# unilight/seq2seq-vc

Measured on AMD Instinct MI355X. Metric: mel-frames/sec (train), higher is better.
Workload: dtype bf16; 1 GPU; VTN egs/arctic/vc1 (vtn.v1.yaml) training step: fwd+Seq2SeqLoss+bwd+clip+Adam+WarmupLR; batch_per_gpu=32, global_batch=32, T_src=256, T_tgt=256, mel_dim=80, parallelism=dp1, split_backward=False, hip_graph=True, backward_stages=1

## Files before the change

### include/s2svc_hip.h

```cpp
#ifndef S2SVC_HIP_H
#define S2SVC_HIP_H
#include <stdint.h>
#ifdef __cplusplus
extern "C" {
#endif

const char* s2svc_last_error(void);
int s2svc_abi_version(void);
int s2svc_launch_floor(int workgroups, int threads, void* sink_1024_words, void* stream);

int s2svc_event_create(void** out );
int s2svc_event_destroy(void* ev);
int s2svc_event_record(void* ev, void* stream);
int s2svc_stream_wait_event(void* stream, void* ev);

enum { S2SVC_LAYOUT_KC = 0,
       S2SVC_LAYOUT_RC = 1 };
enum { S2SVC_OP_DENSE = 0,
       S2SVC_OP_CONV1D = 1,
       S2SVC_OP_CONV2D_S2 = 2,
       S2SVC_OP_TCONV2D_S2 = 3 };

typedef struct {
  const void* ptr;
// ... 121 lines not shown
  int32_t k;
  int32_t reserved_;
} s2svc_scalar_terms;
int s2svc_weighted_sum(const s2svc_scalar_terms* terms , float* out, void* stream);
int s2svc_weighted_sum_bwd(const s2svc_scalar_terms* grads , const float* g, void* stream);
int s2svc_scalars_axpy(const s2svc_scalar_terms* terms , float beta, float* acc, void* stream);
int s2svc_fill_zero(void* p, int64_t nbytes, void* stream);
int s2svc_seed_advance(uint64_t* seed, uint64_t inc, void* stream);
int s2svc_pad_cols(int dtype, int64_t rows, int N, int ldo, const void* in, void* out, void* stream);
int s2svc_decoder_input(int out_dtype, int B, int Tin, int r, int D, int64_t ys_batch_stride, const float* ys, void* out, void* stream);
int s2svc_append_eos(int B, int T, int64_t ldx, const int64_t* xs, const int32_t* lens, int64_t eos, int64_t pad, int64_t* out, void* stream);
int s2svc_copy_rows(int dtype, int64_t rows, int D, int64_t lds, const void* src, void* out, void* stream);
int s2svc_stop_labels(int B, int T, int64_t ld_labels, const float* labels, const int32_t* lens, float* out, void* stream);
int s2svc_add_n(int dtype, int64_t n, int k, const void* x0, const void* x1, const void* x2, const void* x3, void* out, void* stream);
int s2svc_add_head_bias(int dtype, int64_t rows, int D, const void* q, const float* u, const float* v, void* qu, void* qv,
                        void* stream);
int s2svc_add_head_bias_ld(int dtype, int64_t rows, int D, const void* q, int64_t ldq, const float* u, const float* v, void* qu,
                           void* qv, void* stream);
int s2svc_add_rows(int dtype, int64_t rows, int D, const void* a, int64_t lda, const void* b, int64_t ldb, void* out, int64_t ldo,
                   void* stream);
int s2svc_glu_fwd(int dtype, int64_t rows, int C, const void* x, void* y, void* stream);
int s2svc_glu_bwd(int dtype, int64_t rows, int C, const void* x, const void* dy, void* dx, void* stream);
int s2svc_cast(int in_dtype, int out_dtype, int64_t n, const void* x, void* y, void* stream);
int s2svc_gather3(int in_dtype, int out_dtype, int n0, int n1, int n2, int64_t s0, int64_t s1, int64_t s2, int64_t off,
                  const void* in, void* out, void* stream);
typedef struct s2svc_gather3_job {
  const void* in;
  void* out;
  int64_t s0, s1, s2, off;
  int32_t n0, n1, n2;
  int32_t out_dtype;
} s2svc_gather3_job;
int s2svc_gather3_grouped(const s2svc_gather3_job* jobs , int n, void* stream);
int s2svc_permute_inner(int n, int A, int B, const float* src, float* dst, int accumulate, void* stream);
int s2svc_rowscale(int dtype, int64_t rows, int D, const void* x, const float* s, void* out, void* stream);

int s2svc_conv_in1_fwd(int dtype, int B, int Tn, int Fn, int O, const void* x, const float* w, const float* bias, void* y,
                       void* stream);
int s2svc_conv_in1_wgrad(int dtype, int B, int Tn, int Fn, int O, const void* x, const void* dy, const void* y, float* dw,
                         float* db, int accumulate, float* partial, int max_chunks, void* stream);
int s2svc_col2im_s2(int dtype, int B, int T1, int F1, int C, int T2, int F2, const void* dcols, void* dx, void* stream);
int s2svc_interp_nearest(int dtype, int B, int Tin, int Tout, int C, const void* x, void* y, const int32_t* ext_in,
                         const int32_t* ext_out, void* stream);
int s2svc_interp_nearest_bwd(int dtype, int B, int Tin, int Tout, int C, const void* dy, void* dx, const int32_t* ext_in,
                             const int32_t* ext_out, void* stream);
int s2svc_dwconv(int dtype, int B, int Tn, int C, int ks, int dil, const void* x, const float* w, const float* bias,
                 void* y, int flip, void* stream);
int s2svc_dwconv_add(int dtype, int B, int Tn, int C, int ks, int dil, const void* x, const float* w, const float* bias,
                     const void* add, void* y, int flip, void* stream);
int s2svc_dwconv_wgrad(int dtype, int B, int Tn, int C, int ks, int dil, const void* x, const void* dy, float* dw,
                       int accumulate, float* ws, int ws_chunks, void* stream);

int s2svc_convmod_supported(int C, int ks);
int s2svc_convmod_fwd(int B, int Tn, int C, int ks, const void* y2, const float* w, const float* bias, void* z, float eps,
                      float momentum, float* mean, float* rstd, float* run_mean, float* run_var, int64_t* num_batches, float* ws,
                      const int32_t* vlens, void* stream);
int s2svc_bn_swish_apply(int64_t rows, int C, const void* z, const float* mean, const float* rstd, const float* gamma,
                         const float* beta, void* out, int Tn, const int32_t* vlens, void* stream);
int s2svc_convmod_bwd(int B, int Tn, int C, int ks, const void* da, const void* z, const void* y2, const float* w, const float* mean,
                      const float* rstd, const float* gamma, const float* beta, void* dy2, float* sdy, float* sdyx,
                      float* dgamma_acc, float* dbeta_acc, float* ws_stats, float* ws_w, const int32_t* vlens, void* stream);
int s2svc_convmod_wgrad_final(int C, int ks, int chunks, const float* ws_w, float* dw, float* db, int accumulate, void* stream);

int s2svc_bn_stats_vec(int rows, int C, const void* x, float eps, float momentum, float* mean, float* rstd, float* run_mean,
                       float* run_var, int64_t* num_batches, float* ws, int Tn, const int32_t* vlens, void* stream);
int s2svc_bn_act_apply_vec(int rows, int C, const void* x, const float* mean, const float* rstd, const float* gamma, const float* beta,
// ... 195 lines not shown
```

### seq2seq_vc_amd/_lib.py

```python
import ctypes
import os
import subprocess
import sys
from concurrent.futures import ThreadPoolExecutor

_HERE = os.path.dirname(os.path.abspath(__file__))
CSRC = os.path.join(_HERE, "csrc")
LIB_PATH = os.environ.get("S2SVC_LIB") or os.path.join(CSRC, "libs2svc_hip.so")
HIPCC = os.environ.get("HIPCC", "/opt/rocm/bin/hipcc")
ARCH = "gfx950"


def sources():
    return sorted(f for f in os.listdir(CSRC) if f.endswith(".hip"))


DEBUG_EXEC_LIB_PATH = os.path.join(CSRC, "libs2svc_hip_dbgexec.so")


def build_library(force=False, verbose=True, debug_exec=False):
    lib_path = DEBUG_EXEC_LIB_PATH if debug_exec else LIB_PATH
    if not debug_exec and os.environ.get("S2SVC_LIB"):
        lib_path = os.path.join(CSRC, "libs2svc_hip.so")
    srcs = [os.path.join(CSRC, f) for f in sources()]
# ... 49 lines not shown
    if verbose:
        print("[s2svc build]", " ".join(cmd), file=sys.stderr)
    subprocess.run(cmd, check=True)
    return TORCH_OPS_LIB_PATH


c_i32, c_i64, c_f32, c_u64, c_vp = ctypes.c_int32, ctypes.c_int64, ctypes.c_float, ctypes.c_uint64, ctypes.c_void_p


class Operand(ctypes.Structure):
    _fields_ = [("ptr", c_vp), ("ld", c_i64), ("layout", c_i32), ("mode", c_i32), ("C", c_i32), ("T", c_i32),
                ("pad", c_i32), ("T1", c_i32), ("F1", c_i32), ("T2", c_i32), ("F2", c_i32), ("bs0", c_i64),
                ("bs1", c_i64), ("zero_padded", c_i32), ("reserved_", c_i32)]


class GemmDesc(ctypes.Structure):
    _fields_ = [("A", Operand), ("B", Operand), ("C", c_vp), ("ldc", c_i64), ("cbs0", c_i64), ("cbs1", c_i64),
                ("c_dtype", c_i32), ("bias", c_vp), ("res", c_vp), ("ldr", c_i64), ("rbs0", c_i64), ("rbs1", c_i64),
                ("M", c_i32), ("N", c_i32), ("K", c_i32), ("nb0", c_i32), ("nb1", c_i32), ("act", c_i32),
                ("alpha", c_f32), ("dtype", c_i32), ("accumulate", c_i32), ("splitk", c_i32), ("ws", c_vp),
                ("a_rowsum", c_vp), ("a_rowsum_ws", c_vp), ("a_rowsum_accumulate", c_i32), ("tile_hint", c_i32),
                ("emask", c_vp), ("ldm", c_i64), ("drop_p", c_f32), ("emask_mode", c_i32), ("seed_base", c_vp),
                ("seed_off", c_u64), ("c_map", c_i32), ("cm_T1", c_i32), ("cm_F1", c_i32), ("cm_Tc", c_i32), ("cm_Fc", c_i32),
                ("cm_pt", c_i32), ("cm_pf", c_i32), ("reserved3_", c_i32), ("c_pre", c_vp)]


class ScalarTerms(ctypes.Structure):
    _fields_ = [("x", c_vp * 8), ("n", c_i32 * 8), ("w", c_f32 * 8), ("k", c_i32), ("reserved_", c_i32)]


class Gather3Job(ctypes.Structure):
    _fields_ = [("in_", c_vp), ("out", c_vp), ("s0", c_i64), ("s1", c_i64), ("s2", c_i64), ("off", c_i64), ("n0", c_i32),
                ("n1", c_i32), ("n2", c_i32), ("out_dtype", c_i32)]


class ColreduceItem(ctypes.Structure):
    _fields_ = [("dy", c_vp), ("x", c_vp), ("mean", c_vp), ("rstd", c_vp), ("out_sum", c_vp), ("out_dot", c_vp), ("ws", c_vp),
                ("dtype", c_i32), ("rows", c_i32), ("D", c_i32), ("mode", c_i32), ("accumulate", c_i32), ("ws_chunks", c_i32),
                ("scale", c_f32), ("reserved_", c_i32)]


_SIGS = {
    "s2svc_gemm": [ctypes.POINTER(GemmDesc), c_vp],
    "s2svc_gemm_grouped_ok": [c_vp],
    "s2svc_tconv2d_weights": [c_i32, c_i32, c_vp, c_vp, c_vp],
    "s2svc_gemm_grouped": [c_vp, c_i32, c_i32, c_vp],
    "s2svc_gemm_grouped_batched": [c_vp, c_i32, c_vp],
    "s2svc_gemm_wgrad_ok": [c_vp],
    "s2svc_gemm_wgrad_grouped": [c_vp, c_i32, c_vp, c_vp],
    "s2svc_gemm_wgrad_grouped_bg": [c_vp, c_i32, c_vp, c_vp, c_i32],
    "s2svc_gemm_set_w8": [c_i32, c_i32],
    "s2svc_gemm_set_8ph": [c_i32],
    "s2svc_launch_floor": [c_i32, c_i32, c_vp, c_vp],
    "s2svc_event_create": [c_vp],
    "s2svc_event_destroy": [c_vp],
    "s2svc_event_record": [c_vp, c_vp],
    "s2svc_stream_wait_event": [c_vp, c_vp],
    "s2svc_decode_ln_linear_supported": [c_i32, c_i32, c_i32],
    "s2svc_decode_ln_linear": [ctypes.POINTER(GemmDesc), c_vp, c_vp, c_f32, c_vp, c_i64, c_vp],
    "s2svc_length_regulate_index": [c_i32, c_i32, c_i32, c_vp, c_vp, c_vp, c_vp, c_vp],
    "s2svc_length_regulate_fwd": [c_i32, c_i32, c_i32, c_i32, c_i32, c_vp, c_vp, c_f32, c_vp, c_vp],
    "s2svc_length_regulate_bwd": [c_i32, c_i32, c_i32, c_i32, c_i32, c_vp, c_vp, c_vp, c_vp, c_vp],
    "s2svc_attn_durations": [c_i32, c_i32, c_i32, c_vp, c_vp, c_vp, c_vp, c_vp],
    "s2svc_layernorm_fwd": [c_i32, c_i32, c_i32, c_vp, c_vp, c_f32, c_f32, c_vp, c_u64, c_vp, c_vp, c_f32, c_vp, c_vp, c_vp, c_vp, c_vp],
    "s2svc_layernorm_bwd": [c_i32, c_i32, c_i32, c_vp, c_vp, c_vp, c_vp, c_vp, c_vp, c_f32, c_f32, c_vp, c_u64, c_vp, c_vp, c_vp],
    "s2svc_layernorm_bwd_pg_chunks": [c_i32, c_i32, c_i32, c_vp, c_vp, c_vp, c_vp, c_vp, c_vp],
# ... 2 lines not shown
    "s2svc_colreduce": [c_i32, c_i32, c_i32, c_i32, c_vp, c_vp, c_vp, c_vp, c_f32, c_vp, c_vp, c_i32, c_vp, c_i32, c_i32, c_vp, c_vp],
    "s2svc_bn_finalize": [c_i32, c_i32, c_f32, c_f32, c_vp, c_vp, c_vp, c_vp, c_vp, c_vp, c_i32, c_i32, c_vp, c_vp],
    "s2svc_rstd_from_var": [c_i32, c_f32, c_vp, c_vp, c_vp],
    "s2svc_bn_apply": [c_i32, c_i64, c_i32, c_vp, c_vp, c_vp, c_vp, c_vp, c_i32, c_f32, c_vp, c_u64, c_vp, c_vp, c_i32, c_vp, c_vp],
    "s2svc_bn_bwd": [c_i32, c_i64, c_i32, c_vp, c_vp, c_vp, c_vp, c_vp, c_vp, c_vp, c_i32, c_vp, c_i32, c_vp, c_vp],
    "s2svc_bn_stats": [c_i32, c_i32, c_i32, c_vp, c_f32, c_f32, c_vp, c_vp, c_vp, c_vp, c_vp, c_vp, c_i32, c_i32, c_vp, c_vp],
    "s2svc_attn_softmax_fwd": [c_i32, c_i32, c_i32, c_i32, c_i32, c_i32, c_vp, c_vp, c_i32, c_i32, c_i32, c_f32, c_vp, c_i32, c_f32,
                               c_vp, c_u64, c_vp, c_vp, c_vp],
    "s2svc_attn_softmax_bwd": [c_i32, c_i32, c_i32, c_i32, c_i32, c_i32, c_vp, c_vp, c_vp, c_f32, c_f32, c_vp, c_u64, c_vp, c_vp, c_i32,
                               c_i32, c_i32, c_vp],
    "s2svc_act_dropout_fwd": [c_i32, c_i64, c_vp, c_i32, c_f32, c_vp, c_u64, c_vp, c_vp],
    "s2svc_act_dropout_bwd": [c_i32, c_i64, c_vp, c_vp, c_i32, c_f32, c_vp, c_u64, c_vp, c_vp],
    "s2svc_posenc_fwd": [c_i32, c_i64, c_i32, c_i32, c_vp, c_f32, c_vp, c_vp, c_f32, c_vp, c_u64, c_vp, c_vp],
    "s2svc_posenc_bwd": [c_i32, c_i64, c_i32, c_i32, c_vp, c_f32, c_vp, c_f32, c_vp, c_u64, c_vp, c_vp, c_vp, c_vp],
    "s2svc_axpby": [c_i32, c_i64, c_f32, c_vp, c_f32, c_vp, c_vp, c_vp],
    "s2svc_add_n": [c_i32, c_i64, c_i32, c_vp, c_vp, c_vp, c_vp, c_vp, c_vp],
    "s2svc_weighted_sum": [ctypes.POINTER(ScalarTerms), c_vp, c_vp],
    "s2svc_weighted_sum_bwd": [ctypes.POINTER(ScalarTerms), c_vp, c_vp],
    "s2svc_scalars_axpy": [ctypes.POINTER(ScalarTerms), c_f32, c_vp, c_vp],
    "s2svc_fill_zero": [c_vp, c_i64, c_vp],
    "s2svc_seed_advance": [c_vp, c_u64, c_vp],
    "s2svc_pad_cols": [c_i32, c_i64, c_i32, c_i32, c_vp, c_vp, c_vp],
    "s2svc_decoder_input": [c_i32, c_i32, c_i32, c_i32, c_i32, c_i64, c_vp, c_vp, c_vp],
    "s2svc_stop_labels": [c_i32, c_i32, c_i64, c_vp, c_vp, c_vp, c_vp],
    "s2svc_append_eos": [c_i32, c_i32, c_i64, c_vp, c_vp, c_i64, c_i64, c_vp, c_vp],
    "s2svc_copy_rows": [c_i32, c_i64, c_i32, c_i64, c_vp, c_vp, c_vp],
    "s2svc_add_head_bias": [c_i32, c_i64, c_i32, c_vp, c_vp, c_vp, c_vp, c_vp, c_vp],
    "s2svc_add_head_bias_ld": [c_i32, c_i64, c_i32, c_vp, c_i64, c_vp, c_vp, c_vp, c_vp, c_vp],
    "s2svc_add_rows": [c_i32, c_i64, c_i32, c_vp, c_i64, c_vp, c_i64, c_vp, c_i64, c_vp],
    "s2svc_glu_fwd": [c_i32, c_i64, c_i32, c_vp, c_vp, c_vp],
    "s2svc_glu_bwd": [c_i32, c_i64, c_i32, c_vp, c_vp, c_vp, c_vp],
    "s2svc_cast": [c_i32, c_i32, c_i64, c_vp, c_vp, c_vp],
    "s2svc_gather3_grouped": [c_vp, c_i32, c_vp],
    "s2svc_permute_inner": [c_i32, c_i32, c_i32, c_vp, c_vp, c_i32, c_vp],
    "s2svc_gather3": [c_i32, c_i32, c_i32, c_i32, c_i32, c_i64, c_i64, c_i64, c_i64, c_vp, c_vp, c_vp],
    "s2svc_mas": [c_i32, c_i32, c_i32, c_vp, c_vp, c_vp, c_vp, c_vp, c_vp, c_vp, c_vp],
    "s2svc_mas_binloss_bwd": [c_i32, c_i32, c_i32, c_vp, c_vp, c_vp, c_vp, c_vp],
    "s2svc_seq_loss_fwd": [c_i32, c_i32, c_i32, c_i32, c_vp, c_vp, c_vp, c_vp, c_vp, c_vp, c_f32, c_vp, c_vp, c_vp],
    "s2svc_seq_loss_bwd": [c_i32, c_i32, c_i32, c_i32, c_vp, c_vp, c_vp, c_vp, c_vp, c_vp, c_f32, c_vp, c_vp, c_vp, c_vp,
                           c_vp, c_vp, c_vp],
    "s2svc_guided_attn_loss_fwd": [c_i32, c_i32, c_i32, c_i32, c_i32, c_vp, c_vp, c_vp, c_f32, c_f32, c_vp, c_vp, c_vp],
    "s2svc_guided_attn_loss_bwd": [c_i32, c_i32, c_i32, c_i32, c_i32, c_vp, c_vp, c_f32, c_f32, c_vp, c_vp, c_vp, c_vp],
    "s2svc_adam_step": [c_i64, c_vp, c_vp, c_vp, c_vp, c_vp, c_f32, c_f32, c_f32, c_f32, c_f32, c_f32, c_vp, c_vp, c_vp],
    "s2svc_transpose_tiles": [c_i64, c_vp, c_vp, c_vp, c_vp],
    "s2svc_col2im_s2": [c_i32, c_i32, c_i32, c_i32, c_i32, c_i32, c_i32, c_vp, c_vp, c_vp],
    "s2svc_interp_nearest": [c_i32, c_i32, c_i32, c_i32, c_i32, c_vp, c_vp, c_vp, c_vp, c_vp],
    "s2svc_interp_nearest_bwd": [c_i32, c_i32, c_i32, c_i32, c_i32, c_vp, c_vp, c_vp, c_vp, c_vp],
    "s2svc_dwconv": [c_i32, c_i32, c_i32, c_i32, c_i32, c_i32, c_vp, c_vp, c_vp, c_vp, c_i32, c_vp],
    "s2svc_dwconv_add": [c_i32, c_i32, c_i32, c_i32, c_i32, c_i32, c_vp, c_vp, c_vp, c_vp, c_vp, c_i32, c_vp],
    "s2svc_dwconv_wgrad": [c_i32, c_i32, c_i32, c_i32, c_i32, c_i32, c_vp, c_vp, c_vp, c_i32, c_vp, c_i32, c_vp],
    "s2svc_convmod_supported": [c_i32, c_i32],
    "s2svc_convmod_fwd": [c_i32, c_i32, c_i32, c_i32, c_vp, c_vp, c_vp, c_vp, c_f32, c_f32, c_vp, c_vp, c_vp, c_vp, c_vp, c_vp, c_vp, c_vp],
    "s2svc_bn_swish_apply": [c_i64, c_i32, c_vp, c_vp, c_vp, c_vp, c_vp, c_vp, c_i32, c_vp, c_vp],
    "s2svc_convmod_bwd": [c_i32, c_i32, c_i32, c_i32, c_vp, c_vp, c_vp, c_vp, c_vp, c_vp, c_vp, c_vp, c_vp, c_vp, c_vp, c_vp, c_vp, c_vp,
                          c_vp, c_vp, c_vp],
    "s2svc_convmod_wgrad_final": [c_i32, c_i32, c_i32, c_vp, c_vp, c_vp, c_i32, c_vp],
    "s2svc_bn_stats_vec": [c_i32, c_i32, c_vp, c_f32, c_f32, c_vp, c_vp, c_vp, c_vp, c_vp, c_vp, c_i32, c_vp, c_vp],
    "s2svc_bn_act_apply_vec": [c_i32, c_i32, c_vp, c_vp, c_vp, c_vp, c_vp, c_i32, c_f32, c_vp, c_u64, c_vp, c_vp, c_i32, c_vp, c_vp],
    "s2svc_bn_act_bwd_vec": [c_i32, c_i32, c_vp, c_vp, c_vp, c_vp, c_vp, c_vp, c_i32, c_f32, c_vp, c_u64, c_vp, c_vp, c_vp, c_vp, c_vp, c_vp,
                             c_i32, c_vp, c_vp],
    "s2svc_pairwise_l2_logsoftmax": [c_i32, c_i32, c_i32, c_i32, c_i32, c_vp, c_vp, c_vp, c_vp, c_vp, c_vp],
    "s2svc_pairwise_l2_bwd_g": [c_i32, c_i32, c_i32, c_i32, c_vp, c_vp, c_vp, c_vp, c_vp, c_vp, c_vp],
    "s2svc_rowscale": [c_i32, c_i64, c_i32, c_vp, c_vp, c_vp, c_vp],
    "s2svc_gauss_upsample_probs": [c_i32, c_i32, c_i32, c_i32, c_vp, c_vp, c_vp, c_f32, c_vp, c_vp],
    "s2svc_forward_sum": [c_i32, c_i32, c_i32, c_vp, c_vp, c_vp, c_vp, c_f32, c_vp, c_vp, c_vp, c_vp],
    "s2svc_betabinom_prior": [c_i32, c_i32, c_i32, c_vp, c_vp, c_vp, c_vp],
# ... 114 lines not shown
```

### seq2seq_vc_amd/csrc/elementwise.hip

```cpp
#include "common.h"
#include "../../include/s2svc_hip.h"

namespace {

inline int ew_blocks(int64_t total) {
  int64_t b = (total + 255) / 256;
  return (int)(b > 2048 ? 2048 : (b < 1 ? 1 : b));
}
#define EW_LOOP(i, total) \
  for (int64_t i = (int64_t)blockIdx.x * blockDim.x + threadIdx.x; i < (total); i += (int64_t)gridDim.x * blockDim.x)

template <typename T>
__global__ void act_dropout_fwd_kernel(int64_t n, const T* __restrict__ x, int act, float p, const uint64_t* seed_base, uint64_t seed_off, T* __restrict__ y) {
  const uint64_t seed = (seed_base ? *seed_base : 0ull) + seed_off;
  const float inv_keep = p > 0.f ? 1.f / (1.f - p) : 1.f;
  EW_LOOP(i, n) {
    float v = act_apply(ldf(x + i), act);
    if (p > 0.f) v *= dropout_scale(seed, (uint64_t)i, p, inv_keep);
    stf(y + i, v);
  }
}

template <typename T>
__global__ void act_dropout_bwd_kernel(int64_t n, const T* __restrict__ dz, const T* __restrict__ saved, int act, float p,
// ... 266 lines not shown
      int64_t a = 0;
      if (r < R) {
        const int i0 = r / jb.n1, i1 = r - i0 * jb.n1;
        a = jb.off + i0 * jb.s0 + i1 * jb.s1;
      }
#pragma unroll 4
      for (int cc = y; cc < 64; cc += 4) tile[cc][x] = (r < R && c0 + cc < jb.n2) ? in[a + (int64_t)(c0 + cc) * jb.s2] : 0.f;
      __syncthreads();
#pragma unroll 4
      for (int rr = y; rr < 64; rr += 4) {
        const int ro = r0 + rr, c = c0 + x;
        if (ro < R && c < jb.n2) {
          const float v = tile[x][rr];
          const int64_t o = (int64_t)ro * jb.n2 + c;
          if (jb.out_dtype == S2S_F32) ((float*)jb.out)[o] = v;
          else ((bf16_t*)jb.out)[o] = f2bf(v);
        }
      }
      __syncthreads();
    }
    return;
  }
  for (int64_t i = (int64_t)blockIdx.x * blockDim.x + threadIdx.x; i < n; i += (int64_t)gridDim.x * blockDim.x) {
    const int i2 = (int)(i % jb.n2);
    const int64_t t = i / jb.n2;
    const int i1 = (int)(t % jb.n1);
    const int i0 = (int)(t / jb.n1);
    const float v = in[jb.off + i0 * jb.s0 + i1 * jb.s1 + i2 * jb.s2];
    if (jb.out_dtype == S2S_F32) ((float*)jb.out)[i] = v;
    else ((bf16_t*)jb.out)[i] = f2bf(v);
  }
}

template <typename T>
int launch_typed1(int dtype);

}

#define DISPATCH(dtype, KERNEL, total, ...)                                                                  \
  do {                                                                                                       \
    if ((total) == 0) return 0;                                                                              \
    hipStream_t st_ = (hipStream_t)stream;                                                                   \
    if ((dtype) == S2S_F32) hipLaunchKernelGGL(KERNEL<float>, dim3(ew_blocks(total)), dim3(256), 0, st_, __VA_ARGS__); \
    else hipLaunchKernelGGL(KERNEL<bf16_t>, dim3(ew_blocks(total)), dim3(256), 0, st_, __VA_ARGS__);           \
    S2S_CHECK_LAUNCH(#KERNEL);                                                                               \
  } while (0)

#define P(T_, p) ((T_*)(p))

extern "C" int s2svc_act_dropout_fwd(int dtype, int64_t n, const void* x, int act, float p, const uint64_t* seed_base, uint64_t seed_off, void* y,
                                     void* stream) {
  if (n == 0) return 0;
  hipStream_t st = (hipStream_t)stream;
  if (dtype == S2S_F32)
    hipLaunchKernelGGL(act_dropout_fwd_kernel<float>, dim3(ew_blocks(n)), dim3(256), 0, st, n, (const float*)x, act, p, seed_base, seed_off, (float*)y);
  else if (n % 8 == 0 && ((uintptr_t)x) % 16 == 0 && ((uintptr_t)y) % 16 == 0)
    hipLaunchKernelGGL(act_dropout_fwd_vec_kernel, dim3(ew_blocks(n / 8)), dim3(256), 0, st, n / 8, (const bf16_t*)x, act, p, seed_base, seed_off, (bf16_t*)y);
  else
    hipLaunchKernelGGL(act_dropout_fwd_kernel<bf16_t>, dim3(ew_blocks(n)), dim3(256), 0, st, n, (const bf16_t*)x, act, p, seed_base, seed_off, (bf16_t*)y);
  S2S_CHECK_LAUNCH("act_dropout_fwd_kernel");
  return 0;
}

extern "C" int s2svc_act_dropout_bwd(int dtype, int64_t n, const void* dz, const void* saved, int act, float p,
                                     const uint64_t* seed_base, uint64_t seed_off, void* dx, void* stream) {
  if (n == 0) return 0;
// ... 145 lines not shown
  if (in_dtype == S2S_F32 && out_dtype == S2S_BF16)
    hipLaunchKernelGGL((cast_kernel<float, bf16_t>), g, b, 0, st, n, (const float*)x, (bf16_t*)y);
  else if (in_dtype == S2S_BF16 && out_dtype == S2S_F32)
    hipLaunchKernelGGL((cast_kernel<bf16_t, float>), g, b, 0, st, n, (const bf16_t*)x, (float*)y);
  else if (in_dtype == S2S_F32 && out_dtype == S2S_F32)
    hipLaunchKernelGGL((cast_kernel<float, float>), g, b, 0, st, n, (const float*)x, (float*)y);
  else
    hipLaunchKernelGGL((cast_kernel<bf16_t, bf16_t>), g, b, 0, st, n, (const bf16_t*)x, (bf16_t*)y);
  S2S_CHECK_LAUNCH("cast_kernel");
  return 0;
}

extern "C" int s2svc_gather3_grouped(const s2svc_gather3_job* jobs, int n, void* stream) {
  S2S_REQUIRE(n >= 0 && (n == 0 || jobs), "gather3_grouped: bad args");
  hipStream_t st = (hipStream_t)stream;
  for (int i0 = 0; i0 < n; i0 += S2S_GATHER_MAX) {
    gather_jobs g;
    g.n = (n - i0 < S2S_GATHER_MAX) ? n - i0 : S2S_GATHER_MAX;
    int64_t most = 0;
    for (int i = 0; i < g.n; ++i) {
      g.j[i] = jobs[i0 + i];
      S2S_REQUIRE(g.j[i].in && g.j[i].out && g.j[i].n0 > 0 && g.j[i].n1 > 0 && g.j[i].n2 > 0, "gather3_grouped: bad job");
      const int64_t e = (int64_t)g.j[i].n0 * g.j[i].n1 * g.j[i].n2;
      most = e > most ? e : most;
    }
    int bx = (int)((most + 255) / 256);
    if (bx > 2048) bx = 2048;
    hipLaunchKernelGGL(gather3_grouped_kernel, dim3(bx, g.n), dim3(256), 0, st, g);
    S2S_CHECK_LAUNCH("gather3_grouped_kernel");
  }
  return 0;
}

namespace {
__global__ __launch_bounds__(256) void permute_inner_kernel(int A, int B, const float* __restrict__ src, float* __restrict__ dst,
                                                            int accumulate) {
  extern __shared__ float pi_tile[];
  const int64_t base = (int64_t)blockIdx.x * A * B;
  const int n = A * B, pitch = B + 1;
  for (int i = threadIdx.x; i < n; i += 256) {
    const int a = i / B, b = i - a * B;
    pi_tile[a * pitch + b] = src[base + i];
  }
  __syncthreads();
  for (int i = threadIdx.x; i < n; i += 256) {
    const int b = i / A, a = i - b * A;
    const float v = pi_tile[a * pitch + b];
    dst[base + i] = accumulate ? dst[base + i] + v : v;
  }
}
}

extern "C" int s2svc_permute_inner(int n, int A, int B, const float* src, float* dst, int accumulate, void* stream) {
  S2S_REQUIRE(n >= 0 && A > 0 && B > 0 && (n == 0 || (src && dst)), "permute_inner: bad args");
  S2S_REQUIRE((int64_t)A * (B + 1) * 4 <= 64 * 1024, "permute_inner: one A x B matrix must fit 64 KB of LDS");
  if (n == 0) return 0;
  hipLaunchKernelGGL(permute_inner_kernel, dim3((unsigned)n), dim3(256), (size_t)A * (B + 1) * sizeof(float), (hipStream_t)stream, A, B, src, dst,
                     accumulate);
  S2S_CHECK_LAUNCH("permute_inner_kernel");
  return 0;
}

extern "C" int s2svc_gather3(int in_dtype, int out_dtype, int n0, int n1, int n2, int64_t s0, int64_t s1, int64_t s2,
                             int64_t off, const void* in, void* out, void* stream) {
  const int64_t n = (int64_t)n0 * n1 * n2;
  if (n == 0) return 0;
// ... 14 lines not shown
```

### seq2seq_vc_amd/ops/functional.py

```python
import math
import os

import torch
from torch.autograd import Function

from . import kernels as K
from . import kernels_attn as KAT

_STATE = {"dtype": torch.float32}


def set_compute_dtype(dtype):
    if dtype not in (torch.float32, torch.bfloat16):
        raise ValueError("compute dtype must be float32 or bfloat16")
    _STATE["dtype"] = dtype


def compute_dtype():
    return _STATE["dtype"]


def to_compute(x):
    return K.cast(x.contiguous(), _STATE["dtype"])

# ... 1214 lines not shown
        K.gemm(K.operand(x, C, mode=K.CONV2D_S2, C=C, T1=T1, F1=F1, T2=T2, F2=F2), K.operand(wp, 9 * C), B * T2 * F2, O, 9 * C, y,
               in_dtype=dtype, bias=bias, act="relu")
        ctx.params = (weight, bias)
        ctx.save_for_backward(x, y, wp)
        return y

    @staticmethod
    def backward(ctx, dy):
        x, y, wp = ctx.saved_tensors
        weight, bias = ctx.params
        B, T1, F1, C = x.shape
        O = weight.shape[0]
        T2, F2 = y.shape[1], y.shape[2]
        M2 = B * T2 * F2
        dtype = x.dtype
        dy = _c(dy) if ctx.grad_premasked else K.act_dropout_bwd(_c(dy), y, act="relu")
        dw = db = None
        if weight.requires_grad:
            def work():
                dwp = torch.empty((O, 9 * C), dtype=torch.float32, device=x.device)
                rs, racc, dbv = _bias_sink(bias, O)
                tile, sk = K.plan_gemm(O, 9 * C, M2)
                K.gemm(K.operand(dy, O, layout=K.RC),
                       K.operand(x, C, layout=K.RC, mode=K.CONV2D_S2, C=C, T1=T1, F1=F1, T2=T2, F2=F2), O, 9 * C, M2, dwp,
                       in_dtype=dtype, splitk=sk, tile=tile, a_rowsum=rs, a_rowsum_accumulate=racc, wgrad=True)
                return _emit_permuted(weight, dwp, O, 9, C), dbv
            if _slotted(weight, bias):
                _side_run(work, keep=(dy, x))
                _side_flush()
            else:
                dw, db = work()
        dx = None
        if ctx.needs_input_grad[0] and dtype == torch.bfloat16 and O % 8 == 0 and O >= 64 and C % 8 == 0:
            wts = K.tconv2d_weights(weight.detach())
            dx = torch.empty((B, T1, F1, C), dtype=dtype, device=x.device)
            mask = x if ctx.input_is_relu else None
            for cls, wt in enumerate(wts):
                pt, pf = cls >> 1, cls & 1
                Tc, Fc = (T1 - pt + 1) // 2, (F1 - pf + 1) // 2
                if Tc <= 0 or Fc <= 0:
                    continue
                Kc = wt.shape[1]
                K.gemm(K.operand(dy, O, mode=K.TCONV2D_S2, C=O, T1=Tc, F1=Fc, T2=T2, F2=F2, pad=cls), K.operand(wt, Kc),
                       B * Tc * Fc, C, Kc, dx, in_dtype=dtype, c_map=(T1, F1, Tc, Fc, pt, pf), emask=mask)
        elif ctx.needs_input_grad[0]:
            dcols = torch.empty((M2, 9 * C), dtype=dtype, device=x.device)
            K.gemm(K.operand(dy, O), K.operand(wp, 9 * C, layout=K.RC), M2, 9 * C, O, dcols, in_dtype=dtype)
            dx = K.col2im_s2(dcols, B, T1, F1, C, T2, F2)
            if ctx.input_is_relu:
                dx = K.act_dropout_bwd(dx, x, act="relu")
        if not weight.requires_grad and bias is not None and bias.requires_grad:
            db, _ = _reduce_to(bias, None, 0, dy.view(M2, O))
        return dx, dw, db, None, None


def conv2d_s2_relu(x_nhwc, weight, bias, grad_premasked=False, input_is_relu=False):
    return _Conv2dS2.apply(x_nhwc, weight, bias, grad_premasked, input_is_relu)


class _ConvIn1(Function):

    @staticmethod
    def forward(ctx, x, weight, bias, grad_premasked=False):
        x = _c(x)
        y = K.conv_in1_fwd(x, weight.detach(), bias.detach() if bias is not None else None)
        ctx.params = (weight, bias)
        ctx.grad_premasked = grad_premasked
# ... 279 lines not shown
```

### seq2seq_vc_amd/ops/kernels.py

```python
import ctypes
import math
import os

import torch

from .. import _lib

KC, RC = 0, 1
DENSE, CONV1D, CONV2D_S2, TCONV2D_S2 = 0, 1, 2, 3
ACT = {None: 0, "none": 0, "relu": 1, "tanh": 2, "swish": 3, "sigmoid": 4, "gelu": 5}

_DT = {torch.float32: 0, torch.bfloat16: 1}


def dt(t):
    try:
        return _DT[t.dtype if isinstance(t, torch.Tensor) else t]
    except KeyError:
        raise TypeError(f"unsupported dtype {t.dtype if isinstance(t, torch.Tensor) else t}")


def ptr(t):
    return None if t is None else t.data_ptr()

# ... 757 lines not shown
    dx = torch.empty_like(x)
    _lib.check(_lib.lib().s2svc_glu_bwd(dt(x), dy.numel() // C, C, ptr(x), ptr(dy), ptr(dx), stream()), "glu_bwd")
    return dx


def cast(x, dtype, out=None):
    if x.dtype == dtype and out is None:
        return x
    y = torch.empty(x.shape, dtype=dtype, device=x.device) if out is None else out
    if out is not None and (out.dtype != dtype or out.numel() != x.numel() or not out.is_contiguous() or not x.is_contiguous()):
        raise ValueError("cast(out=): contiguous tensors of the target dtype and the same size are required")
    _lib.check(_lib.lib().s2svc_cast(dt(x), _DT[dtype], x.numel(), ptr(x), ptr(y), stream()), "cast")
    return y


def embedding_fwd(idx, w, out_dtype):
    V, D = w.shape
    idx = idx.contiguous()
    y = torch.empty((*idx.shape, D), dtype=out_dtype, device=w.device)
    _lib.check(_lib.lib().s2svc_embedding_fwd(_DT[out_dtype], idx.numel(), D, V, ptr(idx), ptr(w), ptr(y), stream()), "embedding_fwd")
    return y


def embedding_bwd(idx, dy, V, padding_idx, out=None, accumulate=False):
    D = dy.shape[-1]
    dw = torch.empty((V, D), dtype=torch.float32, device=dy.device) if out is None else out
    _lib.check(_lib.lib().s2svc_embedding_bwd(dt(dy), idx.numel(), D, V, ptr(idx), ptr(dy), -1 if padding_idx is None else padding_idx,
                                              ptr(dw), 1 if accumulate else 0, stream()), "embedding_bwd")
    return dw


class PermRegistry(list):
    covered = None


def gather3_cached(weight, n, strides, off, out_dtype):
    reg = getattr(weight, "_s2s_perm_registry", None)
    if reg is None:
        return gather3(weight.detach(), n, strides, off, out_dtype)
    key = (tuple(n), tuple(strides), int(off), out_dtype)
    ent = weight._s2s_perms.get(key)
    if ent is None:
        buf = gather3(weight.detach(), n, strides, off, out_dtype)
        weight._s2s_perms[key] = [buf, weight._version, len(reg)]
        reg.append((weight, key, buf))
        return buf
    if ent[1] != weight._version or (reg.covered is not None and ent[2] >= reg.covered):
        _lib.check(_lib.lib().s2svc_gather3(dt(weight), _DT[out_dtype], n[0], n[1], n[2], strides[0], strides[1], strides[2], off,
                                            ptr(weight), ptr(ent[0]), stream()), "gather3")
        ent[1] = weight._version
    return ent[0]


def gather3_refresh(registry):
    if not registry:
        return
    jobs = (_lib.Gather3Job * len(registry))()
    for jb, (w, (n, st, off, odt), buf) in zip(jobs, registry):
        jb.in_, jb.out = w.data_ptr(), buf.data_ptr()
        jb.s0, jb.s1, jb.s2, jb.off = st[0], st[1], st[2], off
        jb.n0, jb.n1, jb.n2, jb.out_dtype = n[0], n[1], n[2], _DT[odt]
    _lib.check(_lib.lib().s2svc_gather3_grouped(ctypes.addressof(jobs), len(registry), stream()), "gather3_grouped")


def gather3(x, n, strides, off, out_dtype):
    y = torch.empty(n, dtype=out_dtype, device=x.device)
    _lib.check(_lib.lib().s2svc_gather3(dt(x), _DT[out_dtype], n[0], n[1], n[2], strides[0], strides[1], strides[2], off,
                                        ptr(x), ptr(y), stream()), "gather3")
    return y


def permute_inner(src, n, A, Bn, out=None, accumulate=False):
    _need_cuda(src)
    if src.dtype != torch.float32 or not src.is_contiguous():
        raise TypeError("permute_inner: contiguous fp32 source")
    if src.numel() != n * A * Bn:
        raise ValueError(f"permute_inner: source has {src.numel()} elements, n * A * Bn = {n * A * Bn}")
    if out is None:
        out, accumulate = torch.empty(n * A * Bn, dtype=torch.float32, device=src.device), False
    elif out.dtype != torch.float32 or not out.is_contiguous() or out.numel() != n * A * Bn or out.device != src.device:
        raise TypeError(f"permute_inner: `out` must be a contiguous fp32 tensor of {n * A * Bn} elements on {src.device} "
                        f"(got {out.dtype}, contiguous={out.is_contiguous()}, {out.numel()} elements)")
    _lib.check(_lib.lib().s2svc_permute_inner(n, A, Bn, ptr(src), ptr(out), 1 if accumulate else 0, stream()), "permute_inner")
    return out


def permute_inner_ok(A, Bn):
    return A * (Bn + 1) * 4 <= 64 * 1024


def mas(log_p_attn, text_lens_i32, feat_lens_i32):
    B, Tf, Tx = log_p_attn.shape
    dev = log_p_attn.device
    path = torch.empty((B, Tf), dtype=torch.int32, device=dev)
    ds = torch.empty((B, Tx), dtype=torch.float32, device=dev)
    binmean = torch.empty((B,), dtype=torch.float32, device=dev)
    nbytes = _lib.lib().s2svc_mas_ws_bytes(B, Tf, Tx)
# ... 34 lines not shown

def guided_attn_loss_fwd(att, ilens_i32, olens_i32, sigma, alpha):
    B, H, To, Ti = att.shape
    partial = torch.empty(1024, dtype=torch.float32, device=att.device)
    out = torch.empty(2, dtype=torch.float32, device=att.device)
    _lib.check(_lib.lib().s2svc_guided_attn_loss_fwd(dt(att), B, H, To, Ti, ptr(att), ptr(ilens_i32), ptr(olens_i32), sigma, alpha,
                                                     ptr(partial), ptr(out), stream()), "guided_attn_loss_fwd")
    return out


def guided_attn_loss_bwd(shape, dtype, device, ilens_i32, olens_i32, sigma, alpha, stats, gout):
    B, H, To, Ti = shape
    datt = torch.empty(shape, dtype=dtype, device=device)
    _lib.check(_lib.lib().s2svc_guided_attn_loss_bwd(_DT[dtype], B, H, To, Ti, ptr(ilens_i32), ptr(olens_i32), sigma, alpha,
                                                     ptr(stats), ptr(gout), ptr(datt), stream()), "guided_attn_loss_bwd")
    return datt


def adam_step(params, grads, exp_avg, exp_avg_sq, shadow, state, partial, lr, betas=(0.9, 0.999), eps=1e-8, max_norm=1.0,
              warmup_steps=4000.0):
    _lib.check(_lib.lib().s2svc_adam_step(params.numel(), ptr(params), ptr(grads), ptr(exp_avg), ptr(exp_avg_sq), ptr(shadow),
                                          betas[0], betas[1], eps, max_norm, lr, warmup_steps, ptr(partial), ptr(state),
                                          stream()), "adam_step")


def transpose_tiles(tiles, src, dst):
    _lib.check(_lib.lib().s2svc_transpose_tiles(tiles.shape[0], ptr(tiles), ptr(src), ptr(dst), stream()), "transpose_tiles")


def tconv2d_weights(weight):
    O, C = weight.shape[0], weight.shape[1]
    out = torch.empty(9 * C * O, dtype=torch.bfloat16, device=weight.device)
    _lib.check(_lib.lib().s2svc_tconv2d_weights(O, C, ptr(weight), ptr(out), stream()), "tconv2d_weights")
    views, off = [], 0
    for ntaps in (4, 2, 2, 1):
        views.append(out[off:off + C * ntaps * O].view(C, ntaps * O))
        off += C * ntaps * O
    return views


def col2im_s2(dcols, B, T1, F1, C, T2, F2):
    dx = torch.empty((B, T1, F1, C), dtype=dcols.dtype, device=dcols.device)
    _lib.check(_lib.lib().s2svc_col2im_s2(dt(dcols), B, T1, F1, C, T2, F2, ptr(dcols), ptr(dx), stream()), "col2im_s2")
    return dx


def interp_nearest(x, Tout, ext_in=None, ext_out=None):
    B, Tin, C = x.shape
    y = torch.empty((B, Tout, C), dtype=x.dtype, device=x.device)
    _lib.check(_lib.lib().s2svc_interp_nearest(dt(x), B, Tin, Tout, C, ptr(x), ptr(y), ptr(ext_in), ptr(ext_out), stream()), "interp_nearest")
    return y


def interp_nearest_bwd(dy, Tin, ext_in=None, ext_out=None):
    B, Tout, C = dy.shape
    dx = torch.empty((B, Tin, C), dtype=dy.dtype, device=dy.device)
    _lib.check(_lib.lib().s2svc_interp_nearest_bwd(dt(dy), B, Tin, Tout, C, ptr(dy), ptr(dx), ptr(ext_in), ptr(ext_out), stream()),
               "interp_nearest_bwd")
    return dx


def conv_in1_fwd(x, w, bias):
    B, T, Fd = x.shape
    O = w.shape[0]
    y = torch.empty((B, (T - 3) // 2 + 1, (Fd - 3) // 2 + 1, O), dtype=x.dtype, device=x.device)
    _lib.check(_lib.lib().s2svc_conv_in1_fwd(dt(x), B, T, Fd, O, ptr(x), ptr(w), ptr(bias), ptr(y), stream()), "conv_in1_fwd")
    return y


_CI_CHUNKS = 512

# ... 9 lines not shown
```

### seq2seq_vc_amd/optim.py

```python
import collections

import torch

from .ops import kernels as K


Layout = collections.namedtuple("Layout", "params offsets numel groups stacks t_table t_numel")


def _round_up(n, align):
    return (n + align - 1) // align * align


def _source_attention_stacks(model):
    from .modules import Decoder, MultiHeadedAttention
    stacks = []
    for dec in model.modules():
        if not isinstance(dec, Decoder):
            continue
        mods = [layer.src_attn for layer in dec.decoders]
        if not mods or not all(type(m) is MultiHeadedAttention for m in mods):
            continue
        ws = [w for m in mods for w in (m.linear_k.weight, m.linear_v.weight)]
        bs = [b for m in mods for b in (m.linear_k.bias, m.linear_v.bias)]
# ... 137 lines not shown
        tiles = []
        for so, do, rows, cols, owner in plan.t_table:
            t = owner if isinstance(owner, torch.Tensor) else getattr(owner[0], owner[1])[owner[2]]
            t._s2s_bf16_t = self.shadow_t[do:do + rows * cols].view(cols, rows)
            nt = ((rows + 63) // 64) * ((cols + 63) // 64)
            tiles += [(so, do, (rows << 32) | cols, i) for i in range(nt)]
        self.t_tiles = torch.tensor(tiles, dtype=torch.int64, device=dev)
        for g in plan.groups:
            g["module"]._fused["w_q"]._s2s_bf16_t = g["w"][0]._s2s_bf16_t

    def _view(self, off, shape):
        n = 1
        for d in shape:
            n *= d
        t = self.flat_p[off:off + n].view(shape)
        t.requires_grad_(True)
        t._s2s_grad = self.flat_g[off:off + n].view(shape)
        t._s2s_perm_registry = self._perm_jobs
        if self.shadow is not None:
            t._s2s_bf16 = self.shadow[off:off + n].view(shape)
        return t

    def _touch(self):
        self._model.__dict__["_s2s_weight_gen"] = self._model.__dict__.get("_s2s_weight_gen", 0) + 1

    def refresh_shadow(self):
        self._touch()
        if self.shadow is not None:
            self.shadow.copy_(K.cast(self.flat_p, torch.bfloat16))
        self.refresh_derived()

    def refresh_derived(self):
        reg = self._perm_jobs
        K.gather3_refresh(reg)
        if self.flat_p.is_cuda and torch.cuda.is_current_stream_capturing():
            reg.covered = len(reg) if reg.covered is None else min(reg.covered, len(reg))
        if self.shadow_t is not None:
            K.transpose_tiles(self.t_tiles, self.shadow, self.shadow_t)


    def begin_step(self, zero=True):
        if zero:
            self._zero_gradients()

    def join_prologue(self):
        """Empty on purpose: bench.py calls it before the backward pass and is not ours to change; there is nothing to join."""

    def _zero_gradients(self):
        if self.flat_g.is_cuda:
            K.zero_(self.flat_g)
        else:
            self.flat_g.zero_()

    def param_ranges(self, modules):
        mine = set()
        for m in modules:
            mine.update(id(p) for p in (m.parameters() if isinstance(m, torch.nn.Module) else [m]))
        order = sorted(zip(self.offsets, self.params), key=lambda t: t[0])
        ranges, cur = [], None
        for i, (o, p) in enumerate(order):
            end = order[i + 1][0] if i + 1 < len(order) else self.numel
            if id(p) in mine:
                if cur is not None and cur[1] == o:
                    cur[1] = end
                else:
                    cur = [o, end]
                    ranges.append(cur)
            else:
                cur = None
# ... 78 lines not shown
```

Measured before the change: 1.670 million mel-frames/sec.

## Cache transposed-conv class weights and refresh all derived weights in one grouped kernel

Adds a grouped derived-weight refresh kernel that handles both gather3 permutations and tconv2d class-matrix rearrangements. It picks tiled, slab or element-wise paths per job, using LDS transposes for strided reads. The tconv2d backward now reuses a cached bf16 weight buffer that is refreshed once per optimizer step, instead of rebuilding it on every backward call. This removes redundant per-step weight reshuffles and extra launches, but adds version and coverage bookkeeping that must stay correct under graph capture.

```diff
diff --git a/include/s2svc_hip.h b/include/s2svc_hip.h
--- a/include/s2svc_hip.h
+++ b/include/s2svc_hip.h
@@ -177,6 +177,18 @@
   int32_t out_dtype;
 } s2svc_gather3_job;
 int s2svc_gather3_grouped(const s2svc_gather3_job* jobs , int n, void* stream);
+enum { S2SVC_DERIVED_GATHER3 = 0, S2SVC_DERIVED_TCONV2D = 1 };
+typedef struct s2svc_derived_job {
+  const void* in;
+  void* out;
+  int64_t s0, s1, s2, off;
+  int32_t n0, n1, n2;
+  int32_t out_dtype;
+  int32_t kind;
+  int32_t reserved_;
+} s2svc_derived_job;
+int s2svc_derived_refresh(const s2svc_derived_job* jobs , int n, void* stream);
+int s2svc_derived_refresh_plan(const s2svc_derived_job* jobs , int n, int32_t* path , int32_t* units );
 int s2svc_permute_inner(int n, int A, int B, const float* src, float* dst, int accumulate, void* stream);
 int s2svc_rowscale(int dtype, int64_t rows, int D, const void* x, const float* s, void* out, void* stream);
 
diff --git a/seq2seq_vc_amd/_lib.py b/seq2seq_vc_amd/_lib.py
--- a/seq2seq_vc_amd/_lib.py
+++ b/seq2seq_vc_amd/_lib.py
@@ -105,6 +105,11 @@
 class Gather3Job(ctypes.Structure):
     _fields_ = [("in_", c_vp), ("out", c_vp), ("s0", c_i64), ("s1", c_i64), ("s2", c_i64), ("off", c_i64), ("n0", c_i32),
                 ("n1", c_i32), ("n2", c_i32), ("out_dtype", c_i32)]
+
+
+class DerivedJob(ctypes.Structure):
+    _fields_ = [("in_", c_vp), ("out", c_vp), ("s0", c_i64), ("s1", c_i64), ("s2", c_i64), ("off", c_i64), ("n0", c_i32),
+                ("n1", c_i32), ("n2", c_i32), ("out_dtype", c_i32), ("kind", c_i32), ("reserved_", c_i32)]
 
 
 class ColreduceItem(ctypes.Structure):
@@ -173,6 +178,8 @@
     "s2svc_glu_bwd": [c_i32, c_i64, c_i32, c_vp, c_vp, c_vp, c_vp],
     "s2svc_cast": [c_i32, c_i32, c_i64, c_vp, c_vp, c_vp],
     "s2svc_gather3_grouped": [c_vp, c_i32, c_vp],
+    "s2svc_derived_refresh": [c_vp, c_i32, c_vp],
+    "s2svc_derived_refresh_plan": [c_vp, c_i32, c_vp, c_vp],
     "s2svc_permute_inner": [c_i32, c_i32, c_i32, c_vp, c_vp, c_i32, c_vp],
     "s2svc_gather3": [c_i32, c_i32, c_i32, c_i32, c_i32, c_i64, c_i64, c_i64, c_i64, c_vp, c_vp, c_vp],
     "s2svc_mas": [c_i32, c_i32, c_i32, c_vp, c_vp, c_vp, c_vp, c_vp, c_vp, c_vp, c_vp],
diff --git a/seq2seq_vc_amd/csrc/elementwise.hip b/seq2seq_vc_amd/csrc/elementwise.hip
--- a/seq2seq_vc_amd/csrc/elementwise.hip
+++ b/seq2seq_vc_amd/csrc/elementwise.hip
@@ -322,6 +322,137 @@
   }
 }
 
+#define S2S_DERIVED_MAX 48
+#define S2S_DERIVED_LDS (64 * 65)
+enum { DR_ELEMENT = 0, DR_TILE = 1, DR_SLAB = 2, DR_TCONV = 3 };
+struct derived_dev_job {
+  const float* in;
+  void* out;
+  int64_t s0, s1, s2, off;
+  int32_t n0, n1, n2;
+  uint8_t path, out_dtype, i0_fast, ch_log2;
+};
+struct derived_jobs {
+  derived_dev_job j[S2S_DERIVED_MAX];
+  int32_t ubeg[S2S_DERIVED_MAX + 1];
+  int32_t n;
+};
+static_assert(sizeof(derived_jobs) <= 3840, "kernel arguments are limited to 4 KB (the runtime appends its own)");
+
+__device__ __forceinline__ void derived_store(void* out, int out_dtype, int64_t o, float v) {
+  if (out_dtype == S2S_F32) ((float*)out)[o] = v;
+  else ((bf16_t*)out)[o] = f2bf(v);
+}
+
+__device__ __forceinline__ void derived_row(const derived_dev_job& jb, int q, int64_t& src, int64_t& dst) {
+  if (jb.path == DR_TCONV) {
+    const int O = jb.n0, C = jb.n1;
+    const int c = q / 9, k = q - c * 9, kh = k / 3, kw = k - kh * 3;
+    const int pt = kh & 1, pf = kw & 1, nf = 2 - pf, ntaps = (2 - pt) * nf, tap = (kh >> 1) * nf + (kw >> 1);
+    const int first = pt ? (pf ? 8 : 6) : (pf ? 4 : 0);
+    src = q;
+    dst = (int64_t)first * C * O + ((int64_t)c * ntaps + tap) * O;
+    return;
+  }
+  int i0, i1;
+  if (jb.i0_fast) { i1 = q / jb.n0; i0 = q - i1 * jb.n0; }
+  else { i0 = q / jb.n1; i1 = q - i0 * jb.n1; }
+  src = jb.off + i0 * jb.s0 + i1 * jb.s1;
+  dst = ((int64_t)i0 * jb.n1 + i1) * jb.n2;
+}
+
+__global__ __launch_bounds__(256) void derived_refresh_kernel(const derived_jobs g) {
+  __shared__ float lds[S2S_DERIVED_LDS];
+  __shared__ int64_t row_dst[64];
+  const int total = g.ubeg[g.n];
+  int ji = 0;
+  for (int u = blockIdx.x; u < total; u += gridDim.x) {
+    while (g.ubeg[ji + 1] <= u) ++ji;
+    const derived_dev_job& jb = g.j[ji];
+    const int t = u - g.ubeg[ji];
+    const float* in = jb.in;
+    if (jb.path == DR_TILE || jb.path == DR_TCONV) {
+      const bool tconv = jb.path == DR_TCONV;
+      const int R = tconv ? 9 * jb.n1 : jb.n0 * jb.n1, NC = tconv ? jb.n0 : jb.n2;
+      const int64_t cs = tconv ? (int64_t)9 * jb.n1 : jb.s2;
+      const int tc = (NC + 63) / 64;
+      const int r0 = (t / tc) * 64, c0 = (t - (t / tc) * tc) * 64;
+      const int x = threadIdx.x & 63, y = threadIdx.x >> 6;
+      int64_t src = 0, dst = 0;
+      if (r0 + x < R) derived_row(jb, r0 + x, src, dst);
+      if (y == 0) row_dst[x] = dst;
+#pragma unroll
+      for (int k = 0; k < 16; ++k) {
+        const int cc = y + 4 * k;
+        lds[cc * 65 + x] = (r0 + x < R && c0 + cc < NC) ? in[src + (int64_t)(c0 + cc) * cs] : 0.f;
+      }
+      __syncthreads();
+      const int c = c0 + x;
+#pragma unroll
+      for (int k = 0; k < 16; ++k) {
+        const int rr = y + 4 * k;
+        if (r0 + rr < R && c < NC) derived_store(jb.out, jb.out_dtype, row_dst[rr] + c, lds[x * 65 + rr]);
+      }
+      __syncthreads();
+    } else if (jb.path == DR_SLAB) {
+      const int ch = 1 << jb.ch_log2, tc = (jb.n2 + ch - 1) >> jb.ch_log2;
+      const int i0 = t / tc, c0 = (t - i0 * tc) << jb.ch_log2;
+      const int cols = jb.n2 - c0 < ch ? jb.n2 - c0 : ch;
+      const int s2 = (int)jb.s2, span = (cols - 1) * s2 + jb.n1;
+      const int64_t base = jb.off + i0 * jb.s0 + (int64_t)c0 * s2;
+#pragma unroll 4
+      for (int i = threadIdx.x; i < span; i += 256) lds[i] = in[base + i];
+      __syncthreads();
+      const int64_t o0 = (int64_t)i0 * jb.n1 * jb.n2 + c0;
+      for (int i = threadIdx.x; i < jb.n1 * ch; i += 256) {
+        const int i1 = i >> jb.ch_log2, i2 = i & (ch - 1);
+        if (i2 < cols) derived_store(jb.out, jb.out_dtype, o0 + (int64_t)i1 * jb.n2 + i2, lds[i2 * s2 + i1]);
+      }
+      __syncthreads();
+    } else {
+      const int64_t n = (int64_t)jb.n0 * jb.n1 * jb.n2, e0 = (int64_t)t * 4096;
+      for (int k = 0; k < 16; ++k) {
+        const int64_t i = e0 + k * 256 + threadIdx.x;
+        if (i >= n) break;
+        const int i2 = (int)(i % jb.n2);
+        const int64_t r = i / jb.n2;
+        const int i1 = (int)(r % jb.n1), i0 = (int)(r / jb.n1);
+        derived_store(jb.out, jb.out_dtype, i, in[jb.off + i0 * jb.s0 + i1 * jb.s1 + i2 * jb.s2]);
+      }
+    }
+  }
+}
+
+bool derived_plan(const s2svc_derived_job& a, derived_dev_job& d, int64_t& units) {
+  if (!a.in || !a.out || a.n0 <= 0 || a.n1 <= 0 || (a.out_dtype != S2S_F32 && a.out_dtype != S2S_BF16)) return false;
+  d.in = (const float*)a.in; d.out = a.out;
+  d.s0 = a.s0; d.s1 = a.s1; d.s2 = a.s2; d.off = a.off;
+  d.n0 = a.n0; d.n1 = a.n1; d.n2 = a.n2;
+  d.out_dtype = (uint8_t)a.out_dtype; d.i0_fast = 0; d.ch_log2 = 0;
+  if (a.kind == S2SVC_DERIVED_TCONV2D) {
+    if (a.out_dtype != S2S_BF16 || (int64_t)9 * a.n0 * a.n1 >= (int64_t)1 << 31) return false;
+    d.path = DR_TCONV;
+    units = (int64_t)((9 * a.n1 + 63) / 64) * ((a.n0 + 63) / 64);
+    return true;
+  }
+  if (a.kind != S2SVC_DERIVED_GATHER3 || a.n2 <= 0 || (int64_t)a.n0 * a.n1 >= (int64_t)1 << 31) return false;
+  const int64_t a0 = a.s0 < 0 ? -a.s0 : a.s0, a1 = a.s1 < 0 ? -a.s1 : a.s1;
+  if (a.s1 == 1 && a.s2 >= 1 && 63 * a.s2 + a.n1 <= S2S_DERIVED_LDS) {
+    d.path = DR_SLAB;
+    d.ch_log2 = 6;
+    while (d.ch_log2 < 10 && (1 << d.ch_log2) < a.n2 && ((2 << d.ch_log2) - 1) * a.s2 + a.n1 <= S2S_DERIVED_LDS) ++d.ch_log2;
+    units = (int64_t)a.n0 * ((a.n2 + (1 << d.ch_log2) - 1) >> d.ch_log2);
+  } else if (a.n2 >= 32 && a.s2 >= 64 && ((a.s2 > a0 && a.s2 > a1) || a0 == 1 || a1 == 1)) {
+    d.path = DR_TILE;
+    d.i0_fast = a1 != 1 && a0 == 1;
+    units = (((int64_t)a.n0 * a.n1 + 63) / 64) * ((a.n2 + 63) / 64);
+  } else {
+    d.path = DR_ELEMENT;
+    units = ((int64_t)a.n0 * a.n1 * a.n2 + 4095) / 4096;
+  }
+  return true;
+}
+
 template <typename T>
 int launch_typed1(int dtype);
 
@@ -533,6 +664,39 @@
   return 0;
 }
 
+extern "C" int s2svc_derived_refresh_plan(const s2svc_derived_job* jobs, int n, int32_t* path, int32_t* units) {
+  S2S_REQUIRE(n >= 0 && (n == 0 || (jobs && path && units)), "derived_refresh_plan: bad args");
+  for (int i = 0; i < n; ++i) {
+    derived_dev_job d;
+    int64_t u = 0;
+    S2S_REQUIRE(derived_plan(jobs[i], d, u) && u < ((int64_t)1 << 31), "derived_refresh_plan: bad job");
+    path[i] = d.path;
+    units[i] = (int32_t)u;
+  }
+  return 0;
+}
+
+extern "C" int s2svc_derived_refresh(const s2svc_derived_job* jobs, int n, void* stream) {
+  S2S_REQUIRE(n >= 0 && (n == 0 || jobs), "derived_refresh: bad args");
+  for (int i0 = 0; i0 < n; i0 += S2S_DERIVED_MAX) {
+    derived_jobs g = {};
+    g.n = (n - i0 < S2S_DERIVED_MAX) ? n - i0 : S2S_DERIVED_MAX;
+    int64_t total = 0;
+    for (int i = 0; i < g.n; ++i) {
+      int64_t u = 0;
+      S2S_REQUIRE(derived_plan(jobs[i0 + i], g.j[i], u), "derived_refresh: bad job");
+      g.ubeg[i] = (int32_t)total;
+      total += u;
+      S2S_REQUIRE(total < ((int64_t)1 << 31), "derived_refresh: too many work units");
+    }
+    for (int i = g.n; i <= S2S_DERIVED_MAX; ++i) g.ubeg[i] = (int32_t)total;
+    const int bx = total < 2048 ? (int)total : 2048;
+    hipLaunchKernelGGL(derived_refresh_kernel, dim3(bx), dim3(256), 0, (hipStream_t)stream, g);
+    S2S_CHECK_LAUNCH("derived_refresh_kernel");
+  }
+  return 0;
+}
+
 namespace {
 __global__ __launch_bounds__(256) void permute_inner_kernel(int A, int B, const float* __restrict__ src, float* __restrict__ dst,
                                                             int accumulate) {
diff --git a/seq2seq_vc_amd/ops/functional.py b/seq2seq_vc_amd/ops/functional.py
--- a/seq2seq_vc_amd/ops/functional.py
+++ b/seq2seq_vc_amd/ops/functional.py
@@ -1270,7 +1270,7 @@
                 dw, db = work()
         dx = None
         if ctx.needs_input_grad[0] and dtype == torch.bfloat16 and O % 8 == 0 and O >= 64 and C % 8 == 0:
-            wts = K.tconv2d_weights(weight.detach())
+            wts = K.tconv2d_weights_cached(weight)
             dx = torch.empty((B, T1, F1, C), dtype=dtype, device=x.device)
             mask = x if ctx.input_is_relu else None
             for cls, wt in enumerate(wts):
diff --git a/seq2seq_vc_amd/ops/kernels.py b/seq2seq_vc_amd/ops/kernels.py
--- a/seq2seq_vc_amd/ops/kernels.py
+++ b/seq2seq_vc_amd/ops/kernels.py
@@ -813,6 +813,11 @@
 
 class PermRegistry(list):
     covered = None
+    tconv_covered = None
+
+    def __init__(self, *args):
+        super().__init__(*args)
+        self.tconv = []
 
 
 def gather3_cached(weight, n, strides, off, out_dtype):
@@ -844,6 +849,38 @@
     _lib.check(_lib.lib().s2svc_gather3_grouped(ctypes.addressof(jobs), len(registry), stream()), "gather3_grouped")
 
 
+def derived_jobs(gathers, tconvs=()):
+    jobs = (_lib.DerivedJob * (len(gathers) + len(tconvs)))()
+    for jb, (w, (n, st, off, odt), buf) in zip(jobs, gathers):
+        jb.in_, jb.out, jb.kind = w.data_ptr(), buf.data_ptr(), 0
+        jb.s0, jb.s1, jb.s2, jb.off = st[0], st[1], st[2], off
+        jb.n0, jb.n1, jb.n2, jb.out_dtype = n[0], n[1], n[2], _DT[odt]
+    for i, (w, buf) in enumerate(tconvs):
+        jb = jobs[len(gathers) + i]
+        jb.in_, jb.out, jb.kind = w.data_ptr(), buf.data_ptr(), 1
+        jb.n0, jb.n1, jb.n2, jb.out_dtype = w.shape[0], w.shape[1], 1, _DT[torch.bfloat16]
+    return jobs
+
+
+def derived_refresh(gathers, tconvs=()):
+    if not gathers and not tconvs:
+        return
+    for w, buf in tconvs:
+        if w.dtype != torch.float32 or not w.is_contiguous() or w.dim() != 4 or tuple(w.shape[2:]) != (3, 3) or \
+                buf.dtype != torch.bfloat16 or buf.numel() != w.numel() or not buf.is_contiguous():
+            raise ValueError("derived_refresh: a class-matrix job takes a contiguous fp32 (O, C, 3, 3) weight and a bf16 buffer of its size")
+    jobs = derived_jobs(gathers, tconvs)
+    _lib.check(_lib.lib().s2svc_derived_refresh(ctypes.addressof(jobs), len(jobs), stream()), "derived_refresh")
+
+
+def derived_refresh_plan(gathers, tconvs=()):
+    jobs = derived_jobs(gathers, tconvs)
+    path, units = (ctypes.c_int32 * len(jobs))(), (ctypes.c_int32 * len(jobs))()
+    _lib.check(_lib.lib().s2svc_derived_refresh_plan(ctypes.addressof(jobs), len(jobs), ctypes.addressof(path), ctypes.addressof(units)),
+               "derived_refresh_plan")
+    return list(zip(path, units))
+
+
 def gather3(x, n, strides, off, out_dtype):
     y = torch.empty(n, dtype=out_dtype, device=x.device)
     _lib.check(_lib.lib().s2svc_gather3(dt(x), _DT[out_dtype], n[0], n[1], n[2], strides[0], strides[1], strides[2], off,
@@ -944,11 +981,34 @@
     O, C = weight.shape[0], weight.shape[1]
     out = torch.empty(9 * C * O, dtype=torch.bfloat16, device=weight.device)
     _lib.check(_lib.lib().s2svc_tconv2d_weights(O, C, ptr(weight), ptr(out), stream()), "tconv2d_weights")
+    return _tconv2d_views(out, O, C)
+
+
+def _tconv2d_views(out, O, C):
     views, off = [], 0
     for ntaps in (4, 2, 2, 1):
         views.append(out[off:off + C * ntaps * O].view(C, ntaps * O))
         off += C * ntaps * O
     return views
+
+
+def tconv2d_weights_cached(weight):
+    reg = getattr(weight, "_s2s_perm_registry", None)
+    if reg is None or not hasattr(weight, "_s2s_perms"):
+        return tconv2d_weights(weight.detach())
+    O, C = weight.shape[0], weight.shape[1]
+    ent = weight._s2s_perms.get("tconv2d")
+    if ent is None:
+        buf = torch.empty(9 * C * O, dtype=torch.bfloat16, device=weight.device)
+        _lib.check(_lib.lib().s2svc_tconv2d_weights(O, C, ptr(weight), ptr(buf), stream()), "tconv2d_weights")
+        views = _tconv2d_views(buf, O, C)
+        weight._s2s_perms["tconv2d"] = [buf, weight._version, len(reg.tconv), views]
+        reg.tconv.append((weight, buf))
+        return views
+    if ent[1] != weight._version or (reg.tconv_covered is not None and ent[2] >= reg.tconv_covered):
+        _lib.check(_lib.lib().s2svc_tconv2d_weights(O, C, ptr(weight), ptr(ent[0]), stream()), "tconv2d_weights")
+        ent[1] = weight._version
+    return ent[3]
 
 
 def col2im_s2(dcols, B, T1, F1, C, T2, F2):
diff --git a/seq2seq_vc_amd/optim.py b/seq2seq_vc_amd/optim.py
--- a/seq2seq_vc_amd/optim.py
+++ b/seq2seq_vc_amd/optim.py
@@ -193,9 +193,10 @@
 
     def refresh_derived(self):
         reg = self._perm_jobs
-        K.gather3_refresh(reg)
+        K.derived_refresh(reg, reg.tconv)
         if self.flat_p.is_cuda and torch.cuda.is_current_stream_capturing():
             reg.covered = len(reg) if reg.covered is None else min(reg.covered, len(reg))
+            reg.tconv_covered = len(reg.tconv) if reg.tconv_covered is None else min(reg.tconv_covered, len(reg.tconv))
         if self.shadow_t is not None:
             K.transpose_tiles(self.t_tiles, self.shadow, self.shadow_t)
 
```

New measurement: 1.688 million mel-frames/sec (median of 6 runs). 1.1% higher.
